# myscale/MyScaleDB

Hardware: NVIDIA H100
Metric: QPS @ recall@10>=0.95 (exact: recall 1.0), FLAT brute-force IP top-10, 10M x 768-d bf16, batch 1024 (higher is better)
Workload: dtype bf16

## Files before the change

myscaledb_b200/csrc/capi.cu:

```cuda
#include <algorithm>
#include <array>
#include <atomic>
#include <cstdlib>
#include <cstring>
#include <mutex>
#include <vector>

#include "common.cuh"
#include "kernels.h"

namespace b200 {

thread_local std::string g_error;
thread_local int64_t g_launches = 0;
static thread_local int64_t t_last_rows_scored = 0;

void set_error(const std::string &msg) { g_error = msg; }
int fail(int code, const std::string &msg) {
    g_error = msg;
    return code;
}

static int ensure_device() {
    int n = 0;
    cudaError_t e = cudaGetDeviceCount(&n);
    if (e != cudaSuccess || n == 0) {
        cudaGetLastError();
        return fail(B200_ERR_NO_DEVICE, std::string("no CUDA device visible (") +
                                            (e != cudaSuccess ? cudaGetErrorString(e) : "count = 0") +
                                            "); libb200search has no CPU fallback");
    }
    int dev = 0;
    B200_CUDA_OK(cudaGetDevice(&dev));
    int major = 0;
    B200_CUDA_OK(cudaDeviceGetAttribute(&major, cudaDevAttrComputeCapabilityMajor, dev));
    if (major != 9)
        return fail(B200_ERR_NO_DEVICE, "device compute capability major is " + std::to_string(major) +
                                            "; this library carries sm_90a code only");
    return B200_OK;
}

static int num_sms() {
    int dev = 0, n = 132;
    if (cudaGetDevice(&dev) == cudaSuccess) cudaDeviceGetAttribute(&n, cudaDevAttrMultiProcessorCount, dev);
    return n;
}

struct DevBuf {
    void *p = nullptr;
    size_t cap = 0;
    uint64_t reallocs = 0;
    int reserve(size_t bytes) {
        if (bytes <= cap) return B200_OK;
        if (p) cudaFree(p);
        p = nullptr;
        cap = 0;
        reallocs++;
        size_t want = bytes + bytes / 4 + 256;
        cudaError_t e = cudaMalloc(&p, want);
        if (e != cudaSuccess) {
            cudaGetLastError();
            return fail(B200_ERR_NOMEM, "cudaMalloc(" + std::to_string(want) + ") failed: " + cudaGetErrorString(e));
        }
        cap = want;
        return B200_OK;
    }
    void release() {
        if (p) cudaFree(p);
        p = nullptr;
        cap = 0;
        reallocs++;
    }
    template <typename T>
    T *as() {
        return reinterpret_cast<T *>(p);
    }
};

}

using namespace b200;

struct b200_corpus {
    int metric = 0, dtype = 0, d = 0, d_pad = 0;
    int64_t cap = 0, n = 0;
    int64_t row_bytes = 0;
    void *data = nullptr;
    size_t data_cap_bytes = 0;
    int64_t side_cap_rows = 0;
    bool owns = true;
    float *row_scale = nullptr;
    float *row_bias = nullptr;
    int device = 0;
    int path = 0;
    int sms = 132;
    cudaStream_t stream = nullptr;
    std::mutex mu;
    uint64_t serial = 0;
    uint64_t epoch = 0;
    DevBuf w_raw, w_q32, w_qbf, w_qlo, w_qnorm, w_pk, w_pi, w_lk, w_li, w_alive, w_odis, w_oids, w_stage, w_prog;
    DevBuf w_pf_ids, w_pf_tmp, w_pf_rows, w_pf_side;
    std::array<DevBuf *, 18> workspaces() {
        return {&w_raw, &w_q32, &w_qbf, &w_qlo, &w_qnorm, &w_pk, &w_pi, &w_lk, &w_li, &w_alive, &w_odis, &w_oids, &w_stage, &w_prog,
                &w_pf_ids, &w_pf_tmp, &w_pf_rows, &w_pf_side};
    }
    int prefilter = 0;
    int64_t last_rows_scored = 0;
    void *h_pin = nullptr;
    size_t h_pin_bytes = 0;
    unsigned int *d_tickets = nullptr;
    unsigned int fused_seq = 0;
    int d_tickets_d = 0;
    int fused_enabled = 1;
    int rescore_l2 = 1;
    int last_cg = 0, last_mc = 0, last_grid = 0, last_kernel = 0;
    bool timing = false;
    std::vector<std::pair<cudaEvent_t, cudaEvent_t>> ev_used, ev_free;
    double timed_ms = 0;
    int64_t timed_launches = 0;
};

static void timing_begin(b200_corpus *c, cudaStream_t s, std::pair<cudaEvent_t, cudaEvent_t> &ev) {
    if (!c->timing) return;
    if (c->ev_free.empty()) {
        cudaEventCreate(&ev.first);
        cudaEventCreate(&ev.second);
    } else {
        ev = c->ev_free.back();
        c->ev_free.pop_back();
    }
    cudaEventRecord(ev.first, s);
}
static void timing_drain(b200_corpus *c) {
    for (auto &ev : c->ev_used) {
        float ms = 0;
        if (cudaEventSynchronize(ev.second) == cudaSuccess && cudaEventElapsedTime(&ms, ev.first, ev.second) == cudaSuccess) {
            c->timed_ms += ms;
            c->timed_launches++;
        }
        c->ev_free.push_back(ev);
    }
    c->ev_used.clear();
}
static void timing_end(b200_corpus *c, cudaStream_t s, std::pair<cudaEvent_t, cudaEvent_t> &ev) {
    if (!c->timing) return;
    cudaEventRecord(ev.second, s);
    c->ev_used.push_back(ev);
    if (c->ev_used.size() >= 1024) timing_drain(c);
}

static int corpus_alloc(b200_corpus *c, int64_t rows);
static int corpus_norms(b200_corpus *c, int64_t first, int64_t n);

namespace b200 {
int corpus_metric(const b200_corpus *c) { return c->metric; }
bool corpus_timing_enabled(const b200_corpus *c) { return c->timing; }
int corpus_dim(const b200_corpus *c) { return c->d; }
int64_t corpus_query_row_bytes(const b200_corpus *c) { return c->dtype == B200_DTYPE_BIN ? c->d_pad : (int64_t)c->d * 4; }
uint64_t corpus_serial(const b200_corpus *c) { return c->serial; }
uint64_t corpus_state_epoch(b200_corpus *c) {
    std::lock_guard<std::mutex> lk(c->mu);
    uint64_t e = c->epoch;
    for (DevBuf *b : c->workspaces()) e += b->reallocs;
    return e;
}
const void *corpus_device_rows(const b200_corpus *c) { return c->data; }
int corpus_append_device(b200_corpus *c, const float *d_rows, int64_t n, cudaStream_t s) {
    if (!c || (!d_rows && n > 0) || n < 0) return fail(B200_ERR_INVALID, "bad arguments");
    if (n == 0) return B200_OK;
    std::lock_guard<std::mutex> lk(c->mu);
    B200_CUDA_OK(cudaSetDevice(c->device));
    B200_TRY(corpus_alloc(c, std::max(c->n + n, c->cap)));
    char *dst = reinterpret_cast<char *>(c->data) + c->n * c->row_bytes;
    if (c->dtype == B200_DTYPE_BIN) B200_CUDA_OK(cudaMemcpyAsync(dst, d_rows, (size_t)n * c->row_bytes, cudaMemcpyDeviceToDevice, s));
    else if (c->dtype == B200_DTYPE_BF16) B200_CUDA_OK(launch_f32_to_bf16_rows(d_rows, c->d, dst, c->d_pad, n, s));
    else B200_CUDA_OK(launch_pad_rows_f32(d_rows, c->d, reinterpret_cast<float *>(dst), c->d_pad, n, s));
    B200_CUDA_OK(cudaStreamSynchronize(s));
    B200_TRY(corpus_norms(c, c->n, n));
    B200_CUDA_OK(cudaStreamSynchronize(c->stream));
    c->n += n;
    c->epoch++;
    return B200_OK;
}
int corpus_normalize_rows(b200_corpus *c) {
    if (c->dtype != B200_DTYPE_F32) return fail(B200_ERR_UNSUPPORTED, "normalise: fp32 corpora only");
    B200_CUDA_OK(cudaSetDevice(c->device));
    B200_CUDA_OK(launch_normalize_rows_f32(reinterpret_cast<float *>(c->data), c->d_pad, c->n, c->stream));
    B200_CUDA_OK(cudaStreamSynchronize(c->stream));
    return B200_OK;
}
}

static bool is_float_metric(int m) { return m == B200_METRIC_L2 || m == B200_METRIC_IP || m == B200_METRIC_COSINE; }
static bool is_bin_metric(int m) { return m == B200_METRIC_HAMMING || m == B200_METRIC_JACCARD; }

static int pad_for(int dtype, int d) {
    if (dtype == B200_DTYPE_BF16) return (int)round_up(d, 64);
    if (dtype == B200_DTYPE_F32) return (int)round_up(d, 4);
    return d / 8;
}

extern "C" const char *b200_last_error(void) { return g_error.c_str(); }
extern "C" const char *b200_version(void) { return "b200search 0.1 (sm_90a)"; }

extern "C" int b200_device_count(int *out_n) {
    if (!out_n) return fail(B200_ERR_INVALID, "out_n is null");
    int n = 0;
    if (cudaGetDeviceCount(&n) != cudaSuccess) {
        cudaGetLastError();
        n = 0;
    }
    *out_n = n;
    return B200_OK;
}

extern "C" int b200_set_device(int device) {
    B200_TRY(ensure_device());
    B200_CUDA_OK(cudaSetDevice(device));
    return B200_OK;
}

extern "C" int64_t b200_launch_count(int reset) {
    int64_t v = g_launches;
    if (reset) g_launches = 0;
    return v;
}

extern "C" int b200_corpus_create(int metric, int dtype, int d, int64_t capacity_rows, b200_corpus **out) {
    if (!out) return fail(B200_ERR_INVALID, "out is null");
    *out = nullptr;
    if (d <= 0 || capacity_rows < 0) return fail(B200_ERR_INVALID, "bad d / capacity");
    if (dtype == B200_DTYPE_BIN) {
        if (!is_bin_metric(metric)) return fail(B200_ERR_INVALID, "binary corpus needs HAMMING or JACCARD");
        if (d % 8) return fail(B200_ERR_INVALID, "binary dimension must be a multiple of 8 bits");
    } else if (dtype == B200_DTYPE_F32 || dtype == B200_DTYPE_BF16) {
        if (!is_float_metric(metric)) return fail(B200_ERR_INVALID, "float corpus needs L2, IP or COSINE");
    } else {
        return fail(B200_ERR_INVALID, "unknown dtype");
    }
    B200_TRY(ensure_device());
    b200_corpus *c = new b200_corpus();
    c->metric = metric;
    c->dtype = dtype;
    c->d = d;
    c->d_pad = pad_for(dtype, d);
    c->row_bytes = dtype == B200_DTYPE_BIN ? c->d_pad : (int64_t)c->d_pad * (dtype == B200_DTYPE_BF16 ? 2 : 4);
    c->cap = capacity_rows;
    static std::atomic<uint64_t> next_serial{0};
    c->serial = ++next_serial;
    cudaGetDevice(&c->device);
    c->sms = num_sms();
    if (const char *ev = getenv("B200_GEMM_RESCORE_L2")) c->rescore_l2 = atoi(ev);
    if (const char *ev = getenv("B200_FUSED_SCAN")) c->fused_enabled = atoi(ev);
    cudaError_t e = cudaStreamCreateWithFlags(&c->stream, cudaStreamNonBlocking);
    if (e != cudaSuccess) {
        delete c;
        return fail(B200_ERR_CUDA, std::string("cudaStreamCreate: ") + cudaGetErrorString(e));
// ... 54 lines not shown
}

extern "C" int b200_corpus_append(b200_corpus *c, const void *rows, int64_t n) {
    if (!c || (!rows && n > 0) || n < 0) return fail(B200_ERR_INVALID, "bad arguments");
    if (n == 0) return B200_OK;
    std::lock_guard<std::mutex> lk(c->mu);
    B200_CUDA_OK(cudaSetDevice(c->device));
    B200_TRY(corpus_alloc(c, std::max(c->n + n, c->cap)));
    char *dst = reinterpret_cast<char *>(c->data) + c->n * c->row_bytes;
    if (c->dtype == B200_DTYPE_BIN || (c->dtype == B200_DTYPE_F32 && c->d == c->d_pad)) {
        B200_TRY(staged_h2d(dst, rows, (size_t)n * c->row_bytes, c->device, c->stream));
    } else {
        const int64_t chunk = std::max<int64_t>(1, (int64_t)(256ll << 20) / ((int64_t)c->d * 4));
        for (int64_t off = 0; off < n; off += chunk) {
            const int64_t m = std::min(chunk, n - off);
            B200_TRY(c->w_raw.reserve((size_t)m * c->d * 4));
            B200_TRY(staged_h2d(c->w_raw.p, reinterpret_cast<const float *>(rows) + off * c->d, (size_t)m * c->d * 4, c->device,
                                c->stream));
            char *dd = dst + off * c->row_bytes;
            if (c->dtype == B200_DTYPE_BF16)
                B200_CUDA_OK(launch_f32_to_bf16_rows(c->w_raw.as<float>(), c->d, dd, c->d_pad, m, c->stream));
            else
                B200_CUDA_OK(launch_pad_rows_f32(c->w_raw.as<float>(), c->d, reinterpret_cast<float *>(dd), c->d_pad, m, c->stream));
            B200_CUDA_OK(cudaStreamSynchronize(c->stream));
        }
    }
    B200_TRY(corpus_norms(c, c->n, n));
    B200_CUDA_OK(cudaStreamSynchronize(c->stream));
    c->n += n;
    c->epoch++;
    return B200_OK;
}

extern "C" int b200_corpus_memory_bytes(const b200_corpus *c, uint64_t *out_bytes) {
    if (!c || !out_bytes) return fail(B200_ERR_INVALID, "bad arguments");
    uint64_t b = c->owns ? (uint64_t)c->data_cap_bytes : (uint64_t)c->n * (uint64_t)c->row_bytes;
    if (c->row_scale) b += (uint64_t)std::max(c->side_cap_rows, c->n) * 4;
    if (c->row_bias) b += (uint64_t)std::max(c->side_cap_rows, c->n) * 4;
    *out_bytes = b;
    return B200_OK;
}

extern "C" int b200_corpus_adopt_device(b200_corpus *c, const void *device_rows, int64_t n) {
    if (!c || !device_rows || n < 0) return fail(B200_ERR_INVALID, "bad arguments");
    std::lock_guard<std::mutex> lk(c->mu);
    if (c->data) return fail(B200_ERR_INVALID, "corpus already holds data");
    if (c->dtype != B200_DTYPE_BIN && c->d != c->d_pad)
        return fail(B200_ERR_INVALID, "adopted rows must already be padded (d % 64 == 0 for bf16, d % 4 == 0 for f32)");
    B200_CUDA_OK(cudaSetDevice(c->device));
    c->data = const_cast<void *>(device_rows);
    c->owns = false;
    c->n = n;
    c->cap = n;
    if (c->metric == B200_METRIC_COSINE) B200_CUDA_OK(cudaMalloc(&c->row_scale, (size_t)n * 4 + 256));
    if (c->metric == B200_METRIC_L2 || c->dtype == B200_DTYPE_BIN) B200_CUDA_OK(cudaMalloc(&c->row_bias, (size_t)n * 4 + 256));
    c->side_cap_rows = n;
    c->epoch++;
    B200_TRY(corpus_norms(c, 0, n));
    B200_CUDA_OK(cudaStreamSynchronize(c->stream));
    return B200_OK;
}

extern "C" int b200_corpus_size(const b200_corpus *c, int64_t *out_rows) {
    if (!c || !out_rows) return fail(B200_ERR_INVALID, "null argument");
    *out_rows = c->n;
    return B200_OK;
}

extern "C" int b200_corpus_set_path(b200_corpus *c, int path) {
    if (!c || path < 0 || path > 7) return fail(B200_ERR_INVALID, "path must be 0..7");
    std::lock_guard<std::mutex> lk(c->mu);
    c->path = path >= 2 ? 2 : path;
    c->epoch++;
    return B200_OK;
}

extern "C" int b200_corpus_last_variant(b200_corpus *c, int *kernel, int *cta_group, int *pairs_per_cluster, int *grid) {
    if (!c) return fail(B200_ERR_INVALID, "null corpus");
    std::lock_guard<std::mutex> lk(c->mu);
    if (kernel) *kernel = c->last_kernel;
    if (cta_group) *cta_group = c->last_cg;
    if (pairs_per_cluster) *pairs_per_cluster = c->last_mc;
    if (grid) *grid = c->last_grid;
    return B200_OK;
}

extern "C" int b200_corpus_enable_timing(b200_corpus *c, int on) {
    if (!c) return fail(B200_ERR_INVALID, "null corpus");
    std::lock_guard<std::mutex> lk(c->mu);
    c->timing = on != 0;
    return B200_OK;
}

extern "C" int b200_corpus_kernel_time(b200_corpus *c, int reset, double *out_total_ms, int64_t *out_launches) {
    if (!c || !out_total_ms || !out_launches) return fail(B200_ERR_INVALID, "null argument");
    std::lock_guard<std::mutex> lk(c->mu);
    B200_CUDA_OK(cudaSetDevice(c->device));
    timing_drain(c);
    *out_total_ms = c->timed_ms;
    *out_launches = c->timed_launches;
    if (reset) {
        c->timed_ms = 0;
        c->timed_launches = 0;
    }
    return B200_OK;
}

extern "C" int b200_corpus_free(b200_corpus *c) {
    if (!c) return B200_OK;
    cudaSetDevice(c->device);
    if (c->stream) cudaStreamSynchronize(c->stream);
    if (c->data && c->owns) cudaFree(c->data);
    if (c->row_scale) cudaFree(c->row_scale);
    if (c->row_bias) cudaFree(c->row_bias);
    if (c->h_pin) cudaFreeHost(c->h_pin);
    if (c->d_tickets) cudaFree(c->d_tickets);
    for (DevBuf *b : c->workspaces()) b->release();
    for (auto *v : {&c->ev_used, &c->ev_free})
        for (auto &ev : *v) {
            cudaEventDestroy(ev.first);
            cudaEventDestroy(ev.second);
        }
    if (c->stream) cudaStreamDestroy(c->stream);
    delete c;
    return B200_OK;
}

constexpr int64_t kBinaryTensorMinQB2 = 20480;

constexpr int kGemmSyncSlack = 2;

static int gemm_chunk(b200_corpus *c, GemmTopkParams &gp, int64_t nq_c, int k, int kernel, int out_mode, const float *q_add,
                      int ip_min_quirk, int64_t id_offset, float *d_out_dis, int64_t *d_out_ids, cudaStream_t s) {
    const int nq_pad = (int)round_up(nq_c, 128);
    const int q_tiles = nq_pad / 128;
    int grid = gemm_topk_grid(q_tiles, gp.n, c->sms);
    grid = (grid / q_tiles) * q_tiles;
    if (grid < q_tiles) grid = q_tiles;
    const size_t producers = (size_t)grid * gemm_consumer_warpgroups(kernel == B200_KERNEL_GEMM_TF32X3);
    B200_TRY(c->w_pk.reserve(producers * 128 * k * 4));
    B200_TRY(c->w_pi.reserve(producers * 128 * k * 4));
    gp.part_keys = c->w_pk.as<float>();
    gp.part_ids = c->w_pi.as<uint32_t>();
    {
        B200_TRY(c->w_lk.reserve(producers * 128 * list_cap_for(k) * 4));
        B200_TRY(c->w_li.reserve(producers * 128 * list_cap_for(k) * 4));
        gp.list_keys_gmem = c->w_lk.as<float>();
        gp.list_ids_gmem = c->w_li.as<uint32_t>();
    }
    gp.nq_pad = nq_pad;
    gp.nq_valid = (int)nq_c;
    gp.k = k;
    gp.q_tiles = q_tiles;
    if (q_tiles > 1) {
        B200_TRY(c->w_prog.reserve((size_t)grid * 4));
        B200_CUDA_OK(cudaMemsetAsync(c->w_prog.p, 0, (size_t)grid * 4, s));
        gp.progress = c->w_prog.as<int>();
        gp.sync_slack = kGemmSyncSlack;
    }
    const char *detail = nullptr;
    std::pair<cudaEvent_t, cudaEvent_t> ev;
    timing_begin(c, s, ev);
    cudaError_t e = kernel == B200_KERNEL_GEMM_TF32X3 ? launch_gemm3_topk(gp, grid, s, &detail)
                    : kernel == B200_KERNEL_GEMM_B1  ? launch_gemm_b1_topk(gp, grid, s, &detail)
                                                     : launch_gemm_topk(gp, grid, s, &detail);
    timing_end(c, s, ev);
    c->last_kernel = kernel;
    c->last_cg = 1; c->last_mc = 1; c->last_grid = grid;
    if (e != cudaSuccess)
        return fail(B200_ERR_CUDA, std::string("gemm_topk launch: ") + (detail ? detail : cudaGetErrorString(e)));
    MergeParams mp{};
    mp.in_keys = gp.part_keys;
    mp.in_ids = gp.part_ids;
    mp.list_stride = (int64_t)nq_pad * k;
    mp.q_stride = k;
    mp.n_lists = (int)(producers / q_tiles);
    mp.k_in = k;
    mp.k = k;
    mp.nq = nq_c;
    mp.out_mode = out_mode;
    mp.q_add = q_add;
    mp.ip_min_quirk = ip_min_quirk;
    mp.id_offset = id_offset;
    mp.out_dis = d_out_dis;
    mp.out_ids = d_out_ids;
    B200_CUDA_OK(launch_topk_merge(mp, false, s));
    return B200_OK;
}

static int resolved_path(const b200_corpus *c, int64_t nq, int k) {
    if (c->path != 0) return c->path;
    if (c->dtype == B200_DTYPE_BIN) {
        const bool tc_rows = c->row_bytes % 16 == 0, tc_exact = c->d < (1 << 24);
        return (tc_rows && tc_exact && nq >= ceil_div(kBinaryTensorMinQB2, c->row_bytes * c->row_bytes)) ? 2 : 1;
    }
    const int64_t min_nq = c->metric == B200_METRIC_L2 ? 20 : (c->dtype == B200_DTYPE_BF16 ? 2 : 5);
    return (nq >= min_nq && k <= (c->dtype == B200_DTYPE_BF16 ? 1024 : 256)) ? 2 : 1;
}

struct RowsView {
    const void *data;
    int64_t n;
    const float *row_scale, *row_bias;
};
static RowsView full_rows(const b200_corpus *c) { return {c->data, c->n, c->row_scale, c->row_bias}; }

static int search_core(b200_corpus *c, const RowsView &r, const void *d_queries, int64_t nq, int k, const uint8_t *d_alive,
                       int64_t id_offset, int ip_min_quirk, float *d_out_dis, int64_t *d_out_ids, cudaStream_t s) {
    if (k <= 0) return fail(B200_ERR_INVALID, "k must be positive");
    if (nq == 0) return B200_OK;
    if (r.n >= (int64_t)0xffffffffll) return fail(B200_ERR_UNSUPPORTED, "corpus shards are limited to 2^32 - 1 rows");
    const int sms = c->sms;
    c->last_rows_scored = t_last_rows_scored = r.n;

    if (c->dtype == B200_DTYPE_BIN) {
        if (k > 1024) return fail(B200_ERR_UNSUPPORTED, "k > 1024 not supported on the binary scan path");
        const bool tc_rows = c->row_bytes % 16 == 0, tc_exact = c->d < (1 << 24);
        int path = resolved_path(c, nq, k);
        if (path == 2 && !tc_rows)
            return fail(B200_ERR_UNSUPPORTED, "binary tensor-core path needs rows of a multiple of 16 bytes (d % 128 == 0 bits); "
                                              "this corpus has " + std::to_string(c->row_bytes) + "-byte rows");
        if (path == 2 && !tc_exact) return fail(B200_ERR_UNSUPPORTED, "binary tensor-core path needs d < 2^24 bits");
        if (r.n == 0) path = 1;
        const bool jaccard = c->metric == B200_METRIC_JACCARD;
        if (path == 1) {
            int blocks_x = (int)std::min<int64_t>(std::max<int64_t>(1, ceil_div(r.n, 256)), std::max<int64_t>(1, (2 * sms) / std::max<int64_t>(1, std::min<int64_t>(nq, 2 * sms))));
            B200_TRY(c->w_pk.reserve((size_t)nq * blocks_x * k * 4));
            B200_TRY(c->w_pi.reserve((size_t)nq * blocks_x * k * 4));
            BinaryScanParams bp{};
            bp.corpus = reinterpret_cast<const uint8_t *>(r.data);
            bp.queries = reinterpret_cast<const uint8_t *>(d_queries);
            bp.alive = d_alive;
            bp.part_keys = c->w_pk.as<float>();
            bp.part_ids = c->w_pi.as<uint32_t>();
            bp.n = r.n;
            bp.nq = nq;
            bp.nbytes = c->d_pad;
            bp.k = k;
            bp.jaccard = jaccard;
            std::pair<cudaEvent_t, cudaEvent_t> ev;
            timing_begin(c, s, ev);
            B200_CUDA_OK(launch_binary_scan(bp, blocks_x, s));
            timing_end(c, s, ev);
            c->last_kernel = B200_KERNEL_SCAN; c->last_cg = 0; c->last_mc = 0; c->last_grid = blocks_x;
            MergeParams mp{};
            mp.in_keys = bp.part_keys;
            mp.in_ids = bp.part_ids;
            mp.list_stride = k;
            mp.q_stride = (int64_t)blocks_x * k;
            mp.n_lists = blocks_x;
            mp.k_in = k;
            mp.k = k;
            mp.nq = nq;
            mp.out_mode = kOutKey;
            mp.id_offset = id_offset;
            mp.out_dis = d_out_dis;
            mp.out_ids = d_out_ids;
            B200_CUDA_OK(launch_topk_merge(mp, false, s));
            return B200_OK;
        }
        const int64_t QCHUNK = 1024;
        for (int64_t qb = 0; qb < nq; qb += QCHUNK) {
            const int64_t nq_c = std::min(QCHUNK, nq - qb);
            const int64_t nq_pad = round_up(nq_c, 128);
            B200_TRY(c->w_qbf.reserve((size_t)nq_pad * c->row_bytes));
            B200_CUDA_OK(cudaMemsetAsync(c->w_qbf.p, 0, (size_t)nq_pad * c->row_bytes, s));
            B200_CUDA_OK(cudaMemcpyAsync(c->w_qbf.p, reinterpret_cast<const uint8_t *>(d_queries) + qb * c->row_bytes,
                                         (size_t)nq_c * c->row_bytes, cudaMemcpyDeviceToDevice, s));
            B200_TRY(c->w_qnorm.reserve((size_t)nq_pad * 4));
            B200_CUDA_OK(launch_popc_rows(c->w_qbf.as<uint8_t>(), c->row_bytes, nq_c, c->w_qnorm.as<float>(), s));
            GemmTopkParams gp{};
            gp.corpus_bf16 = r.data;
            gp.queries_bf16 = c->w_qbf.p;
            gp.row_bias = r.row_bias;
            gp.n = r.n;
            gp.scale_const = jaccard ? 1.f : -2.f;
            gp.alive = d_alive;
            gp.q_popc = jaccard ? c->w_qnorm.as<float>() : nullptr;
            gp.jaccard = jaccard;
            gp.d_pad = (int)c->row_bytes;
            B200_TRY(gemm_chunk(c, gp, nq_c, k, B200_KERNEL_GEMM_B1, jaccard ? kOutKey : kOutAddQ, jaccard ? nullptr : c->w_qnorm.as<float>(),
                                0, id_offset, d_out_dis + qb * k, d_out_ids + qb * k, s));
        }
        return B200_OK;
    }

    int path = resolved_path(c, nq, k);
    if (r.n == 0) path = 1;
    if (path == 1 && k > 2048) return fail(B200_ERR_UNSUPPORTED, "k > 2048 not supported on the scan path");
    if (path == 2 && k > 1024) return fail(B200_ERR_UNSUPPORTED, "k > 1024 not supported on the GEMM path");
    B200_TRY(c->w_q32.reserve((size_t)nq * c->d_pad * 4));
    float *q32 = c->w_q32.as<float>();
    B200_CUDA_OK(launch_pad_rows_f32(reinterpret_cast<const float *>(d_queries), c->d, q32, c->d_pad, nq, s));
    if (c->metric == B200_METRIC_COSINE && path == 1) B200_CUDA_OK(launch_normalize_rows_f32(q32, c->d_pad, nq, s));

    const int out_mode_scan = c->metric == B200_METRIC_L2 ? kOutKey : c->metric == B200_METRIC_IP ? kOutNeg : kOutOnePlus;

    if (path == 1) {
        int qt = nq == 1 ? 1 : nq <= 4 ? 4 : 8;
        while (qt > 1 && scan_smem_bytes(qt, c->d_pad, k) > 100 * 1024) qt = qt == 8 ? 4 : 1;
        if (scan_smem_bytes(qt, c->d_pad, k) > 200 * 1024)
            return fail(B200_ERR_UNSUPPORTED, "d * 4 + 64 * k exceeds the shared-memory budget of the scan kernel");
        const int elems = c->dtype == B200_DTYPE_BF16 ? 8 : 4;
        const int chunks = c->d_pad / elems;
        int group = 1;
        while (group < 32 && group < chunks) group <<= 1;
// ... 521 lines not shown
```

myscaledb_b200/csrc/ip_gemm_sm90.cu:

```cuda
#include <cstdlib>
#include <type_traits>

#include "gemm_common.cuh"

namespace b200 {
namespace gemm {

template <Operand OP>
struct Op {
    using L = Layout<OP>;
    using Acc = typename std::conditional<OP == Operand::B1, int32_t, float>::type;
    static constexpr bool F32X3 = L::F32X3;
    static constexpr int KB = L::KB, MMA_K = L::MMA_K, A_PLANE = L::A_PLANE, B_PLANE = L::B_PLANE, PLANES = L::PLANES;
    static constexpr int WG = gemm_consumer_warpgroups(F32X3);
    static constexpr int THREADS = WG == 1 ? EPI_THREADS + 32 : 3 * EPI_THREADS;
    static constexpr int PRODUCER_REGS = 40, CONSUMER_REGS = 232;
    static constexpr int B_ROWS = WG * HN;
    static constexpr int PASSES = BN / B_ROWS;
    static constexpr int STAGE_BYTES = PLANES * (A_PLANE + WG * B_PLANE);
    static constexpr int TX_BYTES = PLANES * A_PLANE + WG * B_PLANE;
    static constexpr int STAGING_BYTES = 32 * 32 * 4;
    static constexpr int MAX_ST = F32X3 ? 2 : 3;
    static_assert(MAX_ST <= MAX_STAGES, "barrier arrays");
    __host__ __device__ static constexpr int off_staging(int st) { return st * STAGE_BYTES; }
    __host__ __device__ static constexpr int off_bar(int st) { return off_staging(st) + WG * 4 * STAGING_BYTES; }
    __host__ __device__ static constexpr int off_list(int st) { return off_bar(st) + 256; }
    static constexpr int list_bytes(int k_smem) { return k_smem * EPI_THREADS * 8; }
    static size_t smem_bytes(int st, int k_smem) { return (size_t)off_list(st) + (size_t)WG * list_bytes(k_smem) + SMEM_ALIGN_SLACK; }
    static bool lists_fit(int k_smem) { return smem_bytes(2, k_smem) <= (size_t)SMEM_LIMIT; }
    static int stages_for(int k_smem) {
        int st = MAX_ST;
        while (st > 2 && smem_bytes(st, k_smem) > (size_t)SMEM_LIMIT) st--;
        return st;
    }
};

template <int N>
__device__ __forceinline__ void setmaxnreg_inc() { asm volatile("setmaxnreg.inc.sync.aligned.u32 %0;" ::"n"(N)); }
template <int N>
__device__ __forceinline__ void setmaxnreg_dec() { asm volatile("setmaxnreg.dec.sync.aligned.u32 %0;" ::"n"(N)); }

__device__ __forceinline__ void wg_bar(int wg) { asm volatile("bar.sync %0, 128;" ::"r"(wg + 1) : "memory"); }

__device__ __forceinline__ int slot_row(int warp, int slot) { return (slot < 16 ? 0 : 48) + 16 * warp + slot; }

__device__ __forceinline__ float acc_f32(float x) { return x; }
__device__ __forceinline__ float acc_f32(int32_t x) { return __int_as_float(x); }
template <int G, typename T>
__device__ __forceinline__ void group_keys(float (&u)[32], const T (&d0)[64], const T (&d1)[64], bool side, float sc, float bi, int lane) {
#pragma unroll
    for (int i = 0; i < 4; i++) {
        const int x = 4 * (4 * G + i);
        u[2 * i] = acc_f32(d0[x]);
        u[2 * i + 1] = acc_f32(d0[x + 1]);
        u[8 + 2 * i] = acc_f32(d0[x + 2]);
        u[8 + 2 * i + 1] = acc_f32(d0[x + 3]);
        u[16 + 2 * i] = acc_f32(d1[x]);
        u[16 + 2 * i + 1] = acc_f32(d1[x + 1]);
        u[24 + 2 * i] = acc_f32(d1[x + 2]);
        u[24 + 2 * i + 1] = acc_f32(d1[x + 3]);
    }
    if (!side) return;
#pragma unroll
    for (int j = 0; j < 8; j++) {
        const int col = 8 * (j >> 1) + 2 * (lane & 3) + (j & 1);
        const float s = __shfl_sync(0xffffffffu, sc, col), b = __shfl_sync(0xffffffffu, bi, col);
#pragma unroll
        for (int rho = 0; rho < 4; rho++) {
            float &x = u[8 * rho + j];
            x = -fmaf(x, s, b);
        }
    }
}

template <int G = 0, typename T>
__device__ __forceinline__ void group_keys_at(int g, float (&u)[32], const T (&d0)[64], const T (&d1)[64], bool side, const float (&sc)[4],
                                              const float (&bi)[4], int lane) {
    if (g == G) group_keys<G>(u, d0, d1, side, sc[G], bi[G], lane);
    else if constexpr (G + 1 < HN / 32) group_keys_at<G + 1>(g, u, d0, d1, side, sc, bi, lane);
}

__device__ __forceinline__ float quad_rows_max(const float (&m)[4], int lane) {
    const bool b0 = lane & 1, b1 = lane & 2;
    const float s0 = __shfl_xor_sync(0xffffffffu, b0 ? m[0] : m[2], 1);
    const float s1 = __shfl_xor_sync(0xffffffffu, b0 ? m[1] : m[3], 1);
    const float k0 = fmaxf(b0 ? m[2] : m[0], s0), k1 = fmaxf(b0 ? m[3] : m[1], s1);
    const float s = __shfl_xor_sync(0xffffffffu, b1 ? k0 : k1, 2);
    return fmaxf(b1 ? k1 : k0, s);
}

__device__ __forceinline__ void split_tf32(uint32_t x, uint32_t &hi, uint32_t &lo) {
    hi = x & 0xffffe000u;
    const float r = __uint_as_float(x) - __uint_as_float(hi);
    asm("cvt.rna.tf32.f32 %0, %1;" : "=r"(lo) : "f"(r));
}

__global__ void split_tf32_kernel(const float *__restrict__ src, int64_t n_src, int d_pad, float *__restrict__ hi,
                                  float *__restrict__ lo, int64_t n_pad) {
    const int64_t total = n_pad * d_pad;
    for (int64_t i = (int64_t)blockIdx.x * blockDim.x + threadIdx.x; i < total; i += (int64_t)gridDim.x * blockDim.x) {
        const int64_t r = i / d_pad;
        uint32_t h = 0, l = 0;
        if (r < n_src) split_tf32(__float_as_uint(src[i]), h, l);
        hi[i] = __uint_as_float(h);
        lo[i] = __uint_as_float(l);
    }
}

template <Operand OP>
__global__ void __launch_bounds__(Op<OP>::THREADS, 1)
gemm_topk_kernel(const __grid_constant__ CUtensorMap map_q, const __grid_constant__ CUtensorMap map_qlo,
                 const __grid_constant__ CUtensorMap map_c, const GemmTopkParams p) {
    using O = Op<OP>;
    const int STAGES = p.stages;
    extern __shared__ unsigned char smem_dyn[];
    unsigned char *smem = smem_dyn + ((1024u - (smem_u32(smem_dyn) & 1023u)) & 1023u);
    uint64_t *full_bar = reinterpret_cast<uint64_t *>(smem + O::off_bar(STAGES));
    uint64_t *empty_bar = full_bar + MAX_STAGES;

    const int warp = threadIdx.x >> 5, lane = threadIdx.x & 31;
    const int qt = blockIdx.x % p.q_tiles;
    const int worker = blockIdx.x / p.q_tiles;
    const int W = gridDim.x / p.q_tiles;
    const int64_t n_tiles = (p.n + BN - 1) / BN;
    const int kb_count = (p.d_pad + O::KB - 1) / O::KB;

    if (warp == O::WG * 4 && lane == 0) {
        asm volatile("prefetch.tensormap [%0];" ::"l"(reinterpret_cast<uint64_t>(&map_q)) : "memory");
        asm volatile("prefetch.tensormap [%0];" ::"l"(reinterpret_cast<uint64_t>(&map_c)) : "memory");
        for (int i = 0; i < STAGES; i++) {
            mbar_init(&full_bar[i], 1);
            mbar_init(&empty_bar[i], O::WG * 4);
        }
        asm volatile("fence.mbarrier_init.release.cluster;" ::: "memory");
    }
    __syncthreads();

    if (warp >= O::WG * 4) {
        if constexpr (O::WG == 2) setmaxnreg_dec<O::PRODUCER_REGS>();
        if (warp != O::WG * 4) return;
        int stage = 0;
        uint32_t phase = 0;
        int ordinal = 0;
        bool pacing = p.progress != nullptr;
        for (int64_t t = worker; t < n_tiles; t += W, ordinal++) {
            if (pacing) {
                int ok = 1;
                if (lane == 0) {
                    volatile int *prog = p.progress + (size_t)worker * p.q_tiles;
                    prog[qt] = ordinal + 1;
                    int spins = 0;
                    for (int g = 0; g < p.q_tiles; g++)
                        while (prog[g] < ordinal + 1 - p.sync_slack && spins < 256) {
                            __nanosleep(200);
                            spins++;
                        }
                    if (spins >= 256) prog[qt] = 0x7fffffff;
                    ok = spins < 256;
                }
                pacing = __shfl_sync(0xffffffffu, ok, 0) != 0;
            }
            __syncwarp();
            for (int h = 0; h < O::PASSES; h++) {
                for (int kb = 0; kb < kb_count; kb++) {
                    mbar_wait(&empty_bar[stage], phase ^ 1);
                    if (elect_one()) {
                        unsigned char *st = smem + stage * O::STAGE_BYTES;
                        mbar_arrive_expect_tx(&full_bar[stage], O::TX_BYTES);
                        tma_load_2d(&map_q, &full_bar[stage], st, kb * O::KB, qt * BM);
                        if constexpr (O::F32X3) tma_load_2d(&map_qlo, &full_bar[stage], st + O::A_PLANE, kb * O::KB, qt * BM);
                        tma_load_2d(&map_c, &full_bar[stage], st + O::PLANES * O::A_PLANE, kb * O::KB, (int)(t * BN + h * O::B_ROWS));
                    }
                    __syncwarp();
                    if (++stage == STAGES) {
                        stage = 0;
                        phase ^= 1;
                    }
                }
            }
        }
    } else {
        if constexpr (O::WG == 2) setmaxnreg_inc<O::CONSUMER_REGS>();
        const int wg = threadIdx.x / EPI_THREADS;
        const int tid = threadIdx.x % EPI_THREADS;
        const int wwarp = tid >> 5;
        const int qrow = slot_row(wwarp, lane);
        const bool use_side = p.row_scale || p.row_bias || p.alive || p.scale_const != -1.f;
        const bool jaccard = OP == Operand::B1 && p.jaccard;
        float *staging = reinterpret_cast<float *>(smem + O::off_staging(STAGES) + (wg * 4 + wwarp) * O::STAGING_BYTES);
        const uint32_t staging_s = smem_u32(staging);
        const size_t producer = ((size_t)worker * O::WG + wg) * p.q_tiles + qt;
        ThreadTopK list;
        list.n = 0;
        list.worst = 0;
        list.thr_key = (qt * BM + qrow < p.nq_valid) ? FLT_MAX : -FLT_MAX;
        list.thr_id = 0;
        const int list_cap = list_cap_for(p.k);
        if (p.lists_in_smem) {
            unsigned char *lists = smem + O::off_list(STAGES) + wg * O::list_bytes(list_cap);
            list_bind(list, reinterpret_cast<float *>(lists), reinterpret_cast<uint32_t *>(lists + O::list_bytes(list_cap) / 2), tid, p.k);
        } else {
            list_bind(list, p.list_keys_gmem + producer * list_cap * EPI_THREADS, p.list_ids_gmem + producer * list_cap * EPI_THREADS,
                      tid, p.k);
        }
        const int pq = (jaccard && qt * BM + qrow < p.nq_valid) ? (int)p.q_popc[qt * BM + qrow] : 0;
        const uint32_t smem0 = smem_u32(smem);
        int stage = 0;
        uint32_t phase = 0;
        typename O::Acc d0[64], d1[64];
        for (int64_t t = worker; t < n_tiles; t += W) {
            const int64_t n0 = t * BN;
            const bool tail = n0 + BN > p.n;
            for (int pass = 0; pass < O::PASSES; pass++) {
                const int h = O::WG == 1 ? pass : wg;
                float sc[HN / 32] = {}, bi[HN / 32] = {};
                if (use_side) {
#pragma unroll
                    for (int g = 0; g < HN / 32; g++) {
                        const int64_t r = n0 + h * HN + 32 * g + lane;
                        bool ok = r < p.n;
                        if (ok && p.alive) ok = (p.alive[r >> 3] >> (r & 7)) & 1;
                        sc[g] = ok ? (p.row_scale ? p.row_scale[r] : p.scale_const) : 0.f;
                        bi[g] = ok ? (p.row_bias ? p.row_bias[r] : 0.f) : __int_as_float(0x7f800000);
                    }
                }
                int prev = -1;
                for (int kb = 0; kb < kb_count; kb++) {
                    mbar_wait(&full_bar[stage], phase);
                    const uint32_t st = smem0 + stage * O::STAGE_BYTES;
                    if constexpr (O::F32X3) {
                        uint4 *b = reinterpret_cast<uint4 *>(smem + stage * O::STAGE_BYTES + 2 * O::A_PLANE);
                        uint4 *bl = b + O::B_PLANE / 16;
#pragma unroll
                        for (int i = 0; i < O::B_PLANE / 16 / EPI_THREADS; i++) {
                            const uint4 raw = b[tid + i * EPI_THREADS];
                            uint4 hi, lo;
                            split_tf32(raw.x, hi.x, lo.x);
                            split_tf32(raw.y, hi.y, lo.y);
                            split_tf32(raw.z, hi.z, lo.z);
                            split_tf32(raw.w, hi.w, lo.w);
                            b[tid + i * EPI_THREADS] = hi;
                            bl[tid + i * EPI_THREADS] = lo;
                        }
                        asm volatile("fence.proxy.async.shared::cta;" ::: "memory");
                        wg_bar(wg);
                    }
                    wgmma_fence();
                    if constexpr (O::F32X3) {
                        const uint64_t ahi = make_smem_desc(st), alo = make_smem_desc(st + O::A_PLANE);
                        const uint64_t b = make_smem_desc(st + 2 * O::A_PLANE), blo = make_smem_desc(st + 2 * O::A_PLANE + O::B_PLANE);
                        constexpr uint64_t M1 = (64 * 128) >> 4;
#pragma unroll
                        for (int k = 0; k < O::KB / O::MMA_K; k++) {
                            const uint64_t off = (uint64_t)(k * (O::MMA_K * 4 >> 4));
                            const uint32_t acc0 = (kb | k) != 0 ? 1u : 0u;
                            wgmma_tf32_n128(d0, alo + off, b + off, acc0);
                            wgmma_tf32_n128(d1, alo + M1 + off, b + off, acc0);
                            wgmma_tf32_n128(d0, ahi + off, blo + off, 1u);
                            wgmma_tf32_n128(d1, ahi + M1 + off, blo + off, 1u);
                            wgmma_tf32_n128(d0, ahi + off, b + off, 1u);
                            wgmma_tf32_n128(d1, ahi + M1 + off, b + off, 1u);
                        }
                    } else if constexpr (OP == Operand::B1) {
                        const uint64_t a = make_smem_desc(st), b = make_smem_desc(st + O::A_PLANE + wg * O::B_PLANE);
                        constexpr uint64_t M1 = (64 * 128) >> 4;
#pragma unroll
                        for (int k = 0; k < O::KB / O::MMA_K; k++) {
                            const uint64_t off = (uint64_t)(k * (O::MMA_K >> 4));
                            const uint32_t acc0 = (kb | k) != 0 ? 1u : 0u;
                            wgmma_b1_n128(d0, a + off, b + off, acc0);
                            wgmma_b1_n128(d1, a + M1 + off, b + off, acc0);
                        }
                    } else {
                        const uint64_t a = make_smem_desc(st), b = make_smem_desc(st + O::A_PLANE + wg * O::B_PLANE);
                        constexpr uint64_t M1 = (64 * 128) >> 4;
#pragma unroll
                        for (int k = 0; k < O::KB / O::MMA_K; k++) {
                            const uint64_t off = (uint64_t)(k * (O::MMA_K * 2 >> 4));
                            const uint32_t acc0 = (kb | k) != 0 ? 1u : 0u;
                            wgmma_bf16_n128(d0, a + off, b + off, acc0);
                            wgmma_bf16_n128(d1, a + M1 + off, b + off, acc0);
                        }
                    }
                    wgmma_commit();
                    wgmma_wait<1>();
                    if (prev >= 0) {
                        __syncwarp();
                        if (lane == 0) mbar_arrive(&empty_bar[prev]);
                    }
                    prev = stage;
                    if (++stage == STAGES) {
                        stage = 0;
                        phase ^= 1;
                    }
                }
                wgmma_wait<0>();
                __syncwarp();
                if (lane == 0) mbar_arrive(&empty_bar[prev]);
                if constexpr (OP == Operand::B1) {
#pragma unroll
                    for (int i = 0; i < 64; i++) {
                        d0[i] = __float_as_int((float)d0[i]);
                        d1[i] = __float_as_int((float)d1[i]);
                    }
                }
                const float thr = __shfl_sync(0xffffffffu, fminf(list.thr_key, FLT_MAX), (lane >> 2) + 8 * (2 * (lane & 1) + ((lane >> 1) & 1)));
                uint32_t slow = jaccard ? (1u << HN / 32) - 1 : 0;
                if (!jaccard) {
#pragma unroll
                    for (int g = 0; g < HN / 32; g++) {
                        float u[32], m[4];
                        group_keys_at(g, u, d0, d1, use_side, sc, bi, lane);
#pragma unroll
                        for (int rho = 0; rho < 4; rho++) {
                            const float *x = u + 8 * rho;
                            m[rho] = fmaxf(fmaxf(fmaxf(x[0], x[1]), fmaxf(x[2], x[3])), fmaxf(fmaxf(x[4], x[5]), fmaxf(x[6], x[7])));
                        }
                        if (__any_sync(0xffffffffu, quad_rows_max(m, lane) >= -thr)) slow |= 1u << g;
                    }
                }
#pragma unroll 1
                while (slow) {
                    const int g = __ffs(slow) - 1;
                    slow &= slow - 1;
                    float u[32];
                    group_keys_at(g, u, d0, d1, use_side && !jaccard, sc, bi, lane);
#pragma unroll
                    for (int j = 0; j < 8; j++) {
                        const int col = 8 * (j >> 1) + 2 * (lane & 3) + (j & 1);
#pragma unroll
                        for (int rho = 0; rho < 4; rho++) {
                            const uint32_t a = staging_s + 4 * (col * 32 + (((lane >> 2) + 8 * rho) ^ (8 * (lane & 3))));
                            asm volatile("st.shared.f32 [%0], %1;" ::"r"(a), "f"(u[8 * rho + j]) : "memory");
                        }
                    }
                    __syncwarp();
                    float v[32];
#pragma unroll
                    for (int j = 0; j < 32; j++) {
                        const uint32_t a = staging_s + 4 * (j * 32 + (lane ^ (8 * ((j >> 1) & 3))));
                        asm volatile("ld.shared.f32 %0, [%1];" : "=f"(v[j]) : "r"(a) : "memory");
                    }
                    __syncwarp();
                    if (jaccard) {
                        const float s = g == 0 ? sc[0] : g == 1 ? sc[1] : g == 2 ? sc[2] : sc[3];
                        const float b = g == 0 ? bi[0] : g == 1 ? bi[1] : g == 2 ? bi[2] : bi[3];
#pragma unroll
                        for (int j = 0; j < 32; j++) v[j] = jaccard_negkey(v[j], pq, __shfl_sync(0xffffffffu, s, j), __shfl_sync(0xffffffffu, b, j));
                    }
                    epilogue_chunk<32>(list, v, false, nullptr, nullptr, (uint32_t)(n0 + h * HN + 32 * g), tail, p.n, staging + lane);
                    __syncwarp();
                }
            }
        }
        float *ok = p.part_keys + (producer * BM + qrow) * p.k;
        uint32_t *oi = p.part_ids + (producer * BM + qrow) * p.k;
        list_publish(list, ok, oi);
    }
}

static bool encode_map(CUtensorMap *map, const void *base, int64_t rows, int d_pad, int box_rows, Operand op) {
    EncodeTiledFn fn = get_encode_fn();
    if (!fn) return false;
    const int es = op == Operand::TF32X3 ? 4 : op == Operand::BF16 ? 2 : 1;
    const CUtensorMapDataType type = op == Operand::TF32X3 ? CU_TENSOR_MAP_DATA_TYPE_FLOAT32
                                     : op == Operand::BF16 ? CU_TENSOR_MAP_DATA_TYPE_BFLOAT16
                                                           : CU_TENSOR_MAP_DATA_TYPE_UINT8;
    const cuuint64_t dims[2] = {(cuuint64_t)d_pad, (cuuint64_t)rows};
    const cuuint64_t strides[1] = {(cuuint64_t)d_pad * es};
    const cuuint32_t box[2] = {(cuuint32_t)(128 / es), (cuuint32_t)box_rows};
    const cuuint32_t estr[2] = {1, 1};
    return fn(map, type, 2, const_cast<void *>(base), dims, strides, box, estr, CU_TENSOR_MAP_INTERLEAVE_NONE,
              CU_TENSOR_MAP_SWIZZLE_128B, CU_TENSOR_MAP_L2_PROMOTION_L2_256B, CU_TENSOR_MAP_FLOAT_OOB_FILL_NONE) == CUDA_SUCCESS;
}

template <Operand OP>
static cudaError_t launch(const CUtensorMap &map_q, const CUtensorMap &map_qlo, const CUtensorMap &map_c, const GemmTopkParams &p_in,
                          int grid, cudaStream_t s) {
    using O = Op<OP>;
    GemmTopkParams p = p_in;
    const int list_cap = list_cap_for(p.k);
    p.lists_in_smem = O::lists_fit(list_cap) ? 1 : 0;
    const int k_smem = p.lists_in_smem ? list_cap : 0;
    p.stages = O::stages_for(k_smem);
    const size_t smem = O::smem_bytes(p.stages, k_smem);
    auto kern = gemm_topk_kernel<OP>;
    cudaError_t e = cudaFuncSetAttribute(kern, cudaFuncAttributeMaxDynamicSharedMemorySize, (int)smem);
    if (e != cudaSuccess) return e;
    kern<<<grid, O::THREADS, smem, s>>>(map_q, map_qlo, map_c, p);
    g_launches++;
    return cudaGetLastError();
}

}

int gemm_topk_grid(int q_tiles, int64_t n, int num_sms) {
    const int64_t n_tiles = ceil_div(n, gemm::BN);
    int64_t g = (int64_t)q_tiles * (n_tiles < 1 ? 1 : n_tiles);
    if (g > num_sms) g = num_sms;
    if (g < q_tiles) g = q_tiles;
    return (int)g;
}

cudaError_t launch_split_tf32(const float *src, int64_t n_src, int d_pad, float *hi, float *lo, int64_t n_pad, cudaStream_t s) {
    if (n_pad == 0) return cudaSuccess;
    int64_t b = ceil_div(n_pad * d_pad, 256);
    if (b > 132 * 8) b = 132 * 8;
    gemm::split_tf32_kernel<<<(int)b, 256, 0, s>>>(src, n_src, d_pad, hi, lo, n_pad);
    g_launches++;
    return cudaGetLastError();
}

cudaError_t launch_gemm_topk(const GemmTopkParams &p, int grid, cudaStream_t s, const char **err_detail) {
    *err_detail = nullptr;
    if (grid % p.q_tiles != 0) {
        *err_detail = "grid must be a multiple of q_tiles";
        return cudaErrorInvalidValue;
    }
    CUtensorMap map_q, map_c;
    if (!gemm::encode_map(&map_q, p.queries_bf16, p.nq_pad, p.d_pad, gemm::BM, gemm::Operand::BF16) ||
        !gemm::encode_map(&map_c, p.corpus_bf16, p.n, p.d_pad, gemm::Op<gemm::Operand::BF16>::B_ROWS, gemm::Operand::BF16)) {
        *err_detail = "cuTensorMapEncodeTiled failed";
        return cudaErrorInvalidValue;
    }
    return gemm::launch<gemm::Operand::BF16>(map_q, map_q, map_c, p, grid, s);
}

cudaError_t launch_gemm3_topk(const GemmTopkParams &p, int grid, cudaStream_t s, const char **err_detail) {
    *err_detail = nullptr;
    if (grid % p.q_tiles != 0 || !p.queries_lo) {
        *err_detail = "gemm3: grid must be a multiple of q_tiles, queries_lo set";
        return cudaErrorInvalidValue;
    }
    CUtensorMap map_qhi, map_qlo, map_c;
    if (!gemm::encode_map(&map_qhi, p.queries_bf16, p.nq_pad, p.d_pad, gemm::BM, gemm::Operand::TF32X3) ||
        !gemm::encode_map(&map_qlo, p.queries_lo, p.nq_pad, p.d_pad, gemm::BM, gemm::Operand::TF32X3) ||
        !gemm::encode_map(&map_c, p.corpus_bf16, p.n, p.d_pad, gemm::Op<gemm::Operand::TF32X3>::B_ROWS, gemm::Operand::TF32X3)) {
        *err_detail = "cuTensorMapEncodeTiled failed";
        return cudaErrorInvalidValue;
    }
    return gemm::launch<gemm::Operand::TF32X3>(map_qhi, map_qlo, map_c, p, grid, s);
}

cudaError_t launch_gemm_b1_topk(const GemmTopkParams &p, int grid, cudaStream_t s, const char **err_detail) {
    *err_detail = nullptr;
    if (grid % p.q_tiles != 0 || p.d_pad % 16 != 0 || !p.row_bias || (p.jaccard && !p.q_popc)) {
        *err_detail = "gemm b1: grid must be a multiple of q_tiles, rows a multiple of 16 bytes, popcounts set";
        return cudaErrorInvalidValue;
    }
    CUtensorMap map_q, map_c;
    if (!gemm::encode_map(&map_q, p.queries_bf16, p.nq_pad, p.d_pad, gemm::BM, gemm::Operand::B1) ||
        !gemm::encode_map(&map_c, p.corpus_bf16, p.n, p.d_pad, gemm::Op<gemm::Operand::B1>::B_ROWS, gemm::Operand::B1)) {
        *err_detail = "cuTensorMapEncodeTiled failed";
        return cudaErrorInvalidValue;
    }
    return gemm::launch<gemm::Operand::B1>(map_q, map_q, map_c, p, grid, s);
}

}
```

myscaledb_b200/csrc/kernels.h:

```cpp
#pragma once
#include <cuda_runtime.h>
#include <stdint.h>

namespace b200 {

struct ScanParams {
    const void *corpus;
    const float *queries;
    const float *row_scale;
    const uint8_t *alive;
    float *part_keys;
    uint32_t *part_ids;
    int64_t n, nq;
    int64_t row_bytes;
    int d_pad, k, group;
    int l2, bf16;
    int fused;
    int q_dim;
    int cosine;
    int out_mode, ip_min_quirk;
    int64_t id_offset;
    unsigned int *tickets;
    float *out_dis;
    int64_t *out_ids;
    volatile unsigned int *done_flag;
    unsigned int done_value;
    unsigned int *tiles_done;
    int q_inline;
    int stage_cap;
    float qinline[256];
};

struct BinaryScanParams {
    const uint8_t *corpus;
    const uint8_t *queries;
    const uint8_t *alive;
    float *part_keys;
    uint32_t *part_ids;
    int64_t n, nq;
    int nbytes, k, jaccard;
};

enum { kOutKey = 0, kOutNeg = 1, kOutOnePlus = 2, kOutAddQ = 3, kOutCosQ = 4 };

struct MergeParams {
    const void *in_keys;
    const void *in_ids;
    int64_t list_stride, q_stride;
    int64_t id_list_stride;
    int n_lists, k_in, k;
    int64_t nq;
    int descending;
    int tie_mode;
    int32_t *out_list;
    int out_mode;
    int ip_min_quirk;
    const float *q_add;
    int64_t id_offset;
    float *out_dis;
    int64_t *out_ids;
};

size_t scan_smem_bytes(int qt, int d_pad, int k);
cudaError_t launch_flat_scan(const ScanParams &p, int qt, int blocks_x, cudaStream_t s);
cudaError_t launch_binary_scan(const BinaryScanParams &p, int blocks_x, cudaStream_t s);
cudaError_t launch_topk_merge(const MergeParams &p, bool external, cudaStream_t s);
cudaError_t launch_rescore_l2(const void *corpus, int bf16, int64_t row_bytes, int d_pad, const float *queries, int64_t nq, int64_t id_offset,
                              int k, float *dis, int64_t *ids, cudaStream_t s);

struct GemmTopkParams {
    const void *corpus_bf16;
    const void *queries_bf16;
    const void *queries_lo;
    const float *row_scale;
    float scale_const;
    const float *row_bias;
    const uint8_t *alive;
    const float *q_popc;
    int jaccard;
    float *part_keys;
    uint32_t *part_ids;
    float *list_keys_gmem;
    uint32_t *list_ids_gmem;
    int64_t n;
    int nq_pad, d_pad, k;
    int nq_valid;
    int q_tiles;
    int *progress;
    int stages;
    int lists_in_smem;
    int sync_slack;
};
constexpr int kGemmSmemK = 128;
constexpr int list_tourn_min_k = 17;
__host__ __device__ inline int list_tourn_group(int k) { return k <= 64 ? 8 : 16; }
__host__ __device__ inline int list_cap_tourn(int k) { return k + (k + list_tourn_group(k) - 1) / list_tourn_group(k); }
__host__ __device__ inline int list_cap_for(int k) { return k < list_tourn_min_k ? k : list_cap_tourn(k); }
int gemm_topk_grid(int q_tiles, int64_t n, int num_sms);
constexpr int gemm_consumer_warpgroups(bool f32x3) { return f32x3 ? 1 : 2; }
cudaError_t launch_gemm_topk(const GemmTopkParams &p, int grid, cudaStream_t s, const char **err_detail);
cudaError_t launch_split_tf32(const float *src, int64_t n_src, int d_pad, float *hi, float *lo, int64_t n_pad, cudaStream_t s);
cudaError_t launch_gemm3_topk(const GemmTopkParams &p, int grid, cudaStream_t s, const char **err_detail);
cudaError_t launch_gemm_b1_topk(const GemmTopkParams &p, int grid, cudaStream_t s, const char **err_detail);

size_t prefilter_compact_temp_bytes(int64_t n);
cudaError_t launch_prefilter_compact(const uint8_t *d_alive, int64_t n, uint32_t *d_ids, void *temp, cudaStream_t s);
cudaError_t launch_prefilter_gather(const void *rows, int64_t row_bytes, const float *scale, const float *bias, const uint32_t *ids,
                                    int64_t m, void *out_rows, float *out_scale, float *out_bias, cudaStream_t s);
cudaError_t launch_prefilter_map_ids(const uint32_t *alive_ids, int64_t id_offset, int64_t *ids, int64_t count, cudaStream_t s);

int staged_h2d(void *dst, const void *src, size_t bytes, int device, cudaStream_t s);

cudaError_t launch_f32_to_bf16_rows(const float *src, int d, void *dst, int d_pad, int64_t n, cudaStream_t s);
cudaError_t launch_pad_rows_f32(const float *src, int d, float *dst, int d_pad, int64_t n, cudaStream_t s);
cudaError_t launch_row_norms(const void *rows, int bf16, int d_pad, int64_t n, int mode, float *out, cudaStream_t s);
cudaError_t launch_normalize_rows_f32(float *rows, int d_pad, int64_t n, cudaStream_t s);
cudaError_t launch_popc_rows(const uint8_t *rows, int64_t row_bytes, int64_t n, float *out, cudaStream_t s);

}
```

Measured before the change: 39250.

## Share per-query top-k threshold across CTAs via global atomic bound

Adds a per-query global bound buffer, reset to all-ones each search. Each consumer atomically lowers the bound to its list threshold once its list is full, and reads it back (via L2) to tighten its own filter threshold. This lets tiles skip more candidates in the epilogue. It also parallelizes the producer pacing spin across warp lanes with __any_sync. The cost is extra atomics and L2 loads per pass, plus a memset per launch. Correctness depends on bound_encode/decode being order-preserving and on epilogue_chunk accepting the new bound argument, neither of which is shown.

Measured after the change: 41080, median of 6. 4.7% higher.

```diff
diff --git a/myscaledb_b200/csrc/capi.cu b/myscaledb_b200/csrc/capi.cu
--- a/myscaledb_b200/csrc/capi.cu
+++ b/myscaledb_b200/csrc/capi.cu
@@ -98,11 +98,11 @@
     std::mutex mu;
     uint64_t serial = 0;
     uint64_t epoch = 0;
-    DevBuf w_raw, w_q32, w_qbf, w_qlo, w_qnorm, w_pk, w_pi, w_lk, w_li, w_alive, w_odis, w_oids, w_stage, w_prog;
+    DevBuf w_raw, w_q32, w_qbf, w_qlo, w_qnorm, w_pk, w_pi, w_lk, w_li, w_alive, w_odis, w_oids, w_stage, w_prog, w_qb;
     DevBuf w_pf_ids, w_pf_tmp, w_pf_rows, w_pf_side;
-    std::array<DevBuf *, 18> workspaces() {
+    std::array<DevBuf *, 19> workspaces() {
         return {&w_raw, &w_q32, &w_qbf, &w_qlo, &w_qnorm, &w_pk, &w_pi, &w_lk, &w_li, &w_alive, &w_odis, &w_oids, &w_stage, &w_prog,
-                &w_pf_ids, &w_pf_tmp, &w_pf_rows, &w_pf_side};
+                &w_qb, &w_pf_ids, &w_pf_tmp, &w_pf_rows, &w_pf_side};
     }
     int prefilter = 0;
     int64_t last_rows_scored = 0;
@@ -463,6 +463,9 @@
     gp.nq_valid = (int)nq_c;
     gp.k = k;
     gp.q_tiles = q_tiles;
+    B200_TRY(c->w_qb.reserve((size_t)nq_pad * 4));
+    B200_CUDA_OK(cudaMemsetAsync(c->w_qb.p, 0xff, (size_t)nq_pad * 4, s));
+    gp.query_bound = c->w_qb.as<uint32_t>();
     if (q_tiles > 1) {
         B200_TRY(c->w_prog.reserve((size_t)grid * 4));
         B200_CUDA_OK(cudaMemsetAsync(c->w_prog.p, 0, (size_t)grid * 4, s));
diff --git a/myscaledb_b200/csrc/ip_gemm_sm90.cu b/myscaledb_b200/csrc/ip_gemm_sm90.cu
--- a/myscaledb_b200/csrc/ip_gemm_sm90.cu
+++ b/myscaledb_b200/csrc/ip_gemm_sm90.cu
@@ -145,20 +145,21 @@
         bool pacing = p.progress != nullptr;
         for (int64_t t = worker; t < n_tiles; t += W, ordinal++) {
             if (pacing) {
-                int ok = 1;
-                if (lane == 0) {
-                    volatile int *prog = p.progress + (size_t)worker * p.q_tiles;
-                    prog[qt] = ordinal + 1;
-                    int spins = 0;
-                    for (int g = 0; g < p.q_tiles; g++)
-                        while (prog[g] < ordinal + 1 - p.sync_slack && spins < 256) {
-                            __nanosleep(200);
-                            spins++;
-                        }
-                    if (spins >= 256) prog[qt] = 0x7fffffff;
-                    ok = spins < 256;
-                }
-                pacing = __shfl_sync(0xffffffffu, ok, 0) != 0;
+                volatile int *prog = p.progress + (size_t)worker * p.q_tiles;
+                if (lane == 0) prog[qt] = ordinal + 1;
+                __syncwarp();
+                int spins = 0;
+                while (spins < 256) {
+                    bool behind = false;
+                    for (int g = lane; g < p.q_tiles; g += 32) behind |= prog[g] < ordinal + 1 - p.sync_slack;
+                    if (!__any_sync(0xffffffffu, behind)) break;
+                    __nanosleep(200);
+                    spins++;
+                }
+                if (spins >= 256) {
+                    if (lane == 0) prog[qt] = 0x7fffffff;
+                    pacing = false;
+                }
             }
             __syncwarp();
             for (int h = 0; h < O::PASSES; h++) {
@@ -203,7 +204,9 @@
             list_bind(list, p.list_keys_gmem + producer * list_cap * EPI_THREADS, p.list_ids_gmem + producer * list_cap * EPI_THREADS,
                       tid, p.k);
         }
-        const int pq = (jaccard && qt * BM + qrow < p.nq_valid) ? (int)p.q_popc[qt * BM + qrow] : 0;
+        const int q = qt * BM + qrow;
+        const bool live = q < p.nq_valid;
+        const int pq = (jaccard && live) ? (int)p.q_popc[q] : 0;
         const uint32_t smem0 = smem_u32(smem);
         int stage = 0;
         uint32_t phase = 0;
@@ -213,6 +216,7 @@
             const bool tail = n0 + BN > p.n;
             for (int pass = 0; pass < O::PASSES; pass++) {
                 const int h = O::WG == 1 ? pass : wg;
+                const uint32_t bound_u = live ? __ldcg(p.query_bound + q) : 0xffffffffu;
                 float sc[HN / 32] = {}, bi[HN / 32] = {};
                 if (use_side) {
 #pragma unroll
@@ -304,7 +308,8 @@
                         d1[i] = __float_as_int((float)d1[i]);
                     }
                 }
-                const float thr = __shfl_sync(0xffffffffu, fminf(list.thr_key, FLT_MAX), (lane >> 2) + 8 * (2 * (lane & 1) + ((lane >> 1) & 1)));
+                const float bound = bound_u == 0xffffffffu ? FLT_MAX : bound_decode(bound_u);
+                const float thr = __shfl_sync(0xffffffffu, fminf(list.thr_key, bound), (lane >> 2) + 8 * (2 * (lane & 1) + ((lane >> 1) & 1)));
                 uint32_t slow = jaccard ? (1u << HN / 32) - 1 : 0;
                 if (!jaccard) {
 #pragma unroll
@@ -348,9 +353,12 @@
 #pragma unroll
                         for (int j = 0; j < 32; j++) v[j] = jaccard_negkey(v[j], pq, __shfl_sync(0xffffffffu, s, j), __shfl_sync(0xffffffffu, b, j));
                     }
-                    epilogue_chunk<32>(list, v, false, nullptr, nullptr, (uint32_t)(n0 + h * HN + 32 * g), tail, p.n, staging + lane);
+                    epilogue_chunk<32>(list, v, false, nullptr, nullptr, (uint32_t)(n0 + h * HN + 32 * g), tail, p.n, staging + lane,
+                                       bound);
                     __syncwarp();
                 }
+                if (live && list.n == list.k && list.thr_key < bound && fabsf(list.thr_key) <= FLT_MAX)
+                    atomicMin(p.query_bound + q, bound_encode(list.thr_key));
             }
         }
         float *ok = p.part_keys + (producer * BM + qrow) * p.k;
diff --git a/myscaledb_b200/csrc/kernels.h b/myscaledb_b200/csrc/kernels.h
--- a/myscaledb_b200/csrc/kernels.h
+++ b/myscaledb_b200/csrc/kernels.h
@@ -82,6 +82,7 @@
     uint32_t *part_ids;
     float *list_keys_gmem;
     uint32_t *list_ids_gmem;
+    uint32_t *query_bound;
     int64_t n;
     int nq_pad, d_pad, k;
     int nq_valid;
```
